# rasmusab/bayes.js

Hardware: NVIDIA H100
Metric: posterior draws/sec (chains x iters) Normal(mu,sigma) N=1024 at 1/2/4/8 H100 (higher is better)
Workload: dtype f64

## Files before the change

bayes.js_b200/csrc/amwg_jit.cuh:

```cuda
#pragma once
#include <dlfcn.h>
#include <map>
#include <mutex>
#include <sstream>

namespace jit {

struct Insn {
  int pc = 0, next = 0;
  int op = 0, a = 0;
  bool acc = false, store = false;
  int mode[4] = {AMWG_MODE_NONE, AMWG_MODE_NONE, AMWG_MODE_NONE, AMWG_MODE_NONE};
  int inl[4] = {-1, -1, -1, -1};
  int extra[3] = {0, 0, 0};
  int n_extra = 0;
  int term = -1;
  int pops = 0, pushes = 0;
};

static bool has_result(int op) {
  switch (op) {
    case AMWG_OP_ACC: case AMWG_OP_ACC_RANGE: case AMWG_OP_PLATE: case AMWG_OP_LOOP_BEGIN: case AMWG_OP_LOOP_END:
    case AMWG_OP_STORE: case AMWG_OP_END: return false;
    default: return true;
  }
}

static bool decode(const amwg_model* md, int pc, Insn& in, std::string& err) {
  const int32_t* code = md->code;
  const int n = md->n_code;
  auto need = [&](int k) { if (pc + k > n) { err = "program runs past the end of the code"; return false; } return true; };
  in = Insn();
  in.pc = pc;
  if (!need(1)) return false;
  const unsigned w = (unsigned)code[pc++];
  in.op = (int)(w & 0xff);
  in.acc = (w >> 16) & 1;
  in.store = (w & AMWG_STORE_FLAG) != 0;
  in.a = (int)(w >> 18);
  if (in.op < 0 || in.op >= AMWG_OP__COUNT) { err = "unknown opcode"; return false; }
  int used[4] = {0, 0, 0, 0};
  if (in.op == AMWG_OP_PLATE) {
    if (in.a >= md->n_plates) { err = "plate index out of range"; return false; }
    const int kind = md->plates[in.a].kind;
    if (kind == AMWG_PLATE_NORM_IID) { used[0] = used[1] = 1; }
    else if (kind == AMWG_PLATE_BERN_IID || kind == AMWG_PLATE_NORM_GROUPED) { used[0] = 1; }
  } else {
    for (int k = 0; k < 4; ++k) used[k] = ((w >> (8 + 2 * k)) & 3) != AMWG_MODE_NONE;
  }
  for (int k = 3; k >= 0; --k) {
    if (!used[k]) continue;
    const int m = (w >> (8 + 2 * k)) & 3;
    in.mode[k] = m;
    if (m == AMWG_MODE_STACK) in.pops++;
    else if (m == AMWG_MODE_NONE) { err = "plate operand without a mode"; return false; }
    else { if (!need(1)) return false; in.inl[k] = code[pc++]; }
  }
  auto take = [&](int k) { if (!need(k)) return false; for (int j = 0; j < k; ++j) in.extra[in.n_extra++] = code[pc++]; return true; };
  switch (in.op) {
    case AMWG_OP_DATA: if (!take(1)) return false; break;
    case AMWG_OP_DATA_I: if (!take(2)) return false; break;
    case AMWG_OP_COMP_I: if (!take(3)) return false; break;
    case AMWG_OP_PLATE_SS: case AMWG_OP_ACC_RANGE: case AMWG_OP_LOOP_BEGIN: if (!take(1)) return false; break;
    case AMWG_OP_LOOP_END: if (!take(1)) return false; in.pops++; break;
    case AMWG_OP_ACC: case AMWG_OP_STORE: in.pops++; break;
    default: break;
  }
  if (has_result(in.op)) {
    if (in.acc) { if (in.store) { if (!need(1)) return false; in.term = code[pc++]; } }
    else in.pushes = 1;
  } else if (in.op == AMWG_OP_PLATE && in.store) {
    if (!need(1)) return false;
    in.term = code[pc++];
  }
  in.next = pc;
  return true;
}

static bool decode_program(const amwg_model* md, int pc, std::vector<Insn>& out, int* max_depth, std::string& err) {
  out.clear();
  int depth = 0, deepest = 0;
  if (pc < 0 || pc >= md->n_code) { err = "program offset out of range"; return false; }
  for (int guard = 0; guard < md->n_code + 1; ++guard) {
    Insn in;
    if (!decode(md, pc, in, err)) return false;
    depth -= in.pops;
    if (depth < 0) { err = "operand stack underflow"; return false; }
    depth += in.pushes;
    deepest = std::max(deepest, depth);
    out.push_back(in);
    if (in.op == AMWG_OP_END) { if (max_depth) *max_depth = deepest; return true; }
    pc = in.next;
  }
  err = "program has no END";
  return false;
}

static std::string lit(double v) {
  if (v != v) return "CUDART_NAN";
  if (v == INFINITY) return "CUDART_INF";
  if (v == -INFINITY) return "(-CUDART_INF)";
  char buf[64];
  snprintf(buf, sizeof buf, "%a", v);
  std::string s(buf);
  if (v < 0 || (v == 0 && std::signbit(v))) s = "(" + s + ")";
  return s;
}
static std::string istr(long long v) { return std::to_string(v); }
static std::string bits(double v) {
  long long b;
  memcpy(&b, &v, 8);
  return std::to_string(b) + "LL";
}

struct Plan {
  int threads = 128, minblocks = 7;
  int n_res = 0;
  std::vector<int> res_col, res_off, res_bytes;
  std::vector<int> col_smem_off;
  int stream_col = -1;
  int ring_off = 0, ring_stages = 4, ring_tile = 1024;
  int ws_smem = 0, ws_off = 0;
  unsigned smem_bytes = 0;
  std::vector<int> bern_mask_off;
};

struct Source {
  bool full = false;
  std::string generated;
  std::string prelude;
  Plan plan;
};

static const int kMaxGeneratedInsns = 6000;
static const unsigned kResidentBudget = 64u * 1024u;
static const unsigned kJitWsSmemLimit = 20u * 1024u;

struct Emitter {
  std::ostringstream os;
  std::map<std::string, std::string> cse;
  std::vector<std::string> stk;
  std::vector<std::map<std::string, std::string>> scopes;
  int nv = 0;
  std::string tmp(const std::string& rhs) {
    auto it = cse.find(rhs);
    if (it != cse.end()) return it->second;
    std::string name = "v" + std::to_string(nv++);
    os << "    const double " << name << " = " << rhs << ";\n";
    cse[rhs] = name;
    return name;
  }
};

struct Inst {
  std::vector<Insn> ins;
// ... 368 lines not shown
  tables << "__device__ __forceinline__ int jp_type(int p) { return JP_TYPE[p]; }\n"
            "__device__ __forceinline__ int jp_ncomp(int p) { return JP_NCOMP[p]; }\n"
            "__device__ __forceinline__ int jp_dim0(int p) { return JP_DIM0[p]; }\n"
            "__device__ __forceinline__ int jp_off(int p) { return JP_OFF[p]; }\n"
            "__device__ __forceinline__ double jp_lower(int p) { return __longlong_as_double(JP_LOWER[p]); }\n"
            "__device__ __forceinline__ double jp_upper(int p) { return __longlong_as_double(JP_UPPER[p]); }\n";
}


static std::string build_source(const amwg_model* md, const std::vector<double>& consts, unsigned long long n_chains, int sm_count,
                                double norm_c0, Source& src) {
  if (!md->comp_prog || md->n_terms <= 0 || md->stat_prog < 0) return "the model has no pre-evaluated statistics";
  if (md->n_variant_comps > 0) return "variant programs";
  const int D = md->n_comp, P = md->n_params, NT = md->n_terms;
  if (D > 65535 || P > 255) return "too many components / parameters";
  int max_dim0 = 1;
  for (int p = 0; p < P; ++p) {
    if (md->params[p].type == AMWG_BINARY) return "binary parameter";
    if (md->params[p].n_comp > 1) max_dim0 = std::max(max_dim0, std::max(md->params[p].dim0, 2));
  }
  std::string err;

  std::vector<Insn> stat;
  if (!decode_program(md, md->stat_prog, stat, nullptr, err)) return "stat_prog: " + err;
  struct StatEntry { int q, slot, comp; size_t first, last; bool simple; };
  std::vector<StatEntry> entries;
  {
    size_t start = 0;
    for (size_t i = 0; i < stat.size(); ++i) {
      if (stat[i].op == AMWG_OP_END) break;
      if (stat[i].op != AMWG_OP_PLATE_SS) continue;
      StatEntry e{stat[i].a, stat[i].extra[0], -1, start, i, false};
      if (e.q < 0 || e.q >= md->n_plates || md->plates[e.q].kind != AMWG_PLATE_NORM_IID) return "stat_prog refers to a plate that is not NORM_IID";
      if (e.slot < 0 || e.slot >= NT) return "statistic slot out of range";
      if (i == start && stat[i].mode[0] == AMWG_MODE_COMP) { e.simple = true; e.comp = stat[i].inl[0]; if (e.comp < 0 || e.comp >= D) return "component out of range"; }
      entries.push_back(e);
      start = i + 1;
    }
  }
  if (entries.empty()) return "no plate statistics";

  Plan& pl = src.plan;
  pl = Plan();
  pl.col_smem_off.assign(md->n_columns, -1);
  std::vector<char> col_used(md->n_columns, 0);
  for (const auto& e : entries) {
    const int c = md->plates[e.q].col[0];
    if (c < 0 || c >= md->n_columns) return "plate column out of range";
    const amwg_plate& p = md->plates[e.q];
    if (p.iparam[2] < 0 || (long long)p.iparam[2] + p.n > md->columns[c].n) return "plate runs past its column";
    col_used[c] = 1;
  }
  unsigned off = 0;
  std::vector<int> big;
  for (int c = 0; c < md->n_columns; ++c) {
    if (!col_used[c]) continue;
    const unsigned bytes = pad16(std::max<size_t>(sizeof(double) * (size_t)md->columns[c].n, 16));
    if (off + bytes <= kResidentBudget) {
      pl.col_smem_off[c] = (int)off; pl.res_col.push_back(c); pl.res_off.push_back((int)off); pl.res_bytes.push_back((int)bytes);
      off += bytes;
    } else big.push_back(c);
  }
  pl.n_res = (int)pl.res_col.size();
  if (big.size() > 1) return "more than one column exceeds shared memory";
  std::vector<StatEntry> r_entries, s_entries, x_entries;
  for (const auto& e : entries) {
    const int c = md->plates[e.q].col[0];
    const bool resident = pl.col_smem_off[c] >= 0;
    if (e.simple) (resident ? r_entries : s_entries).push_back(e);
    else { if (!resident) return "a plate with an expression mean lies on a streamed column"; x_entries.push_back(e); }
  }
  int s_begin = 0, s_total = 0;
  if (!big.empty()) {
    pl.stream_col = big[0];
    if (s_entries.empty()) return "streamed column without plates";
    std::stable_sort(s_entries.begin(), s_entries.end(), [&](const StatEntry& a, const StatEntry& b) { return md->plates[a.q].iparam[2] < md->plates[b.q].iparam[2]; });
    s_begin = md->plates[s_entries[0].q].iparam[2];
    if (s_begin & 1) return "streamed plates start at an odd offset";
    int cur = s_begin;
    for (const auto& e : s_entries) {
      const amwg_plate& p = md->plates[e.q];
      if (p.iparam[2] != cur || p.n <= 0) return "streamed plates do not tile their column";
      cur += p.n;
    }
    s_total = cur - s_begin;
    pl.ring_off = (int)off;
    off += (unsigned)(pl.ring_stages * pl.ring_tile * 8);
  }
  {
    const size_t per_thread = sizeof(double) * (size_t)(2 * NT + 3 * D) + sizeof(unsigned short) * (size_t)D;
    std::string e = choose_shape(pl, off, per_thread, n_chains, sm_count);
    if (!e.empty()) return e;
  }

  std::ostringstream tables, funcs;
  int table_counter = 0;
  GenCtx gc;
  gc.md = md; gc.consts = &consts; gc.tables = &tables; gc.table_counter = &table_counter;
  std::vector<std::vector<Insn>> progs(D);
  std::map<std::string, std::vector<int>> classes_by_sig;
  std::vector<std::string> sig_order;
  int total_insns = 0;
  for (int c = 0; c < D; ++c) {
    std::vector<Insn> full;
    if (!decode_program(md, md->comp_prog[c], full, nullptr, err)) return "comp_prog: " + err;
    for (const Insn& in : full) if (in.op != AMWG_OP_ACC_RANGE) progs[c].push_back(in);
    std::string sg = signature(progs[c]);
    if (!classes_by_sig.count(sg)) sig_order.push_back(sg);
    classes_by_sig[sg].push_back(c);
  }
  std::vector<int> cls_of(D, 0), mem_of(D, 0);
  funcs << "namespace amwg {\n";
  std::ostringstream step;
  step << "__device__ __forceinline__ bool jit_step(const int c, const double prop, const double coin, double* __restrict__ wk, const unsigned long long ws,\n"
          "                                         double* __restrict__ sp, const unsigned long long ss) {\n";
  bool need_mem = false;
  struct ClassCode { std::string mem, body, stage, commit, hcommit; };
  std::vector<ClassCode> cls_code;
  bool hoist = sig_order.size() > 1;
  int n_cv = 0;
  for (size_t k = 0; k < sig_order.size(); ++k) {
    const std::vector<int>& members = classes_by_sig[sig_order[k]];
    std::vector<Inst> inst;
    for (size_t m = 0; m < members.size(); ++m) {
      Inst it; it.ins = progs[members[m]]; it.moved = members[m];
      inst.push_back(it);
      cls_of[members[m]] = (int)k; mem_of[members[m]] = (int)m;
    }
    ClassCode cc;
    std::string why;
    if (!emit_step_class(gc, inst, cc.body, cc.commit, &total_insns, why)) return "component program: " + why;
    if (total_insns > kMaxGeneratedInsns) return "the component programs are too long to specialise";
    if (cc.commit.empty()) return "a component touches no term";
    if (inst.size() > 1) { cc.mem = "    const int m = JMEM[c];\n"; need_mem = true; }
    std::istringstream lines(cc.commit);
    std::ostringstream stage, commit;
    int i = 0;
    for (std::string ln; std::getline(lines, ln);) {
      const size_t eq = ln.find(") = ");
      const std::string rhs = eq == std::string::npos ? "" : ln.substr(eq + 4);
      const bool named = rhs.size() > 2 && rhs[0] == 'v' && rhs.back() == ';' && rhs.find_first_not_of("0123456789", 1) == rhs.size() - 1;
      if (ln.compare(0, 7, "    TV(") != 0 || eq == std::string::npos) { hoist = false; break; }
      if (rhs.compare(0, 3, "TC(") == 0) { commit << ln << "\n"; continue; }
      if (!named) { hoist = false; break; }
      stage << "    cv[" << i << "] = " << rhs << "\n";
      commit << ln.substr(0, eq + 4) << "cv[" << i << "];\n";
      ++i;
    }
    n_cv = std::max(n_cv, i);
    cc.stage = stage.str();
    cc.hcommit = commit.str();
    cls_code.push_back(cc);
  }
  if (hoist) {
    step << "  double dl = 0.0;\n";
    if (n_cv > 0) step << "  double cv[" << n_cv << "];\n";
    step << "  switch (JCLS[c]) {\n";
    for (size_t k = 0; k < cls_code.size(); ++k) step << "  case " << k << ": {\n" << cls_code[k].mem << cls_code[k].body << cls_code[k].stage << "    break;\n  }\n";
    step << "  default: return false;\n  }\n";
    step << "  if (!(js_exp(dl) > coin)) return false;              // Metropolis accept (mcmc.js:527-534): strict >, NaN rejects\n";
    step << "  ST(c) = prop;\n  switch (JCLS[c]) {\n";
    for (size_t k = 0; k < cls_code.size(); ++k) step << "  case " << k << ": {\n" << cls_code[k].mem << cls_code[k].hcommit << "    break;\n  }\n";
    step << "  }\n  return true;\n}\n";
  }
  if (!hoist && sig_order.size() > 1) step << "  switch (JCLS[c]) {\n";
  for (size_t k = 0; !hoist && k < cls_code.size(); ++k) {
    if (sig_order.size() > 1) step << "  case " << k << ": {\n";
    else step << "  {\n";
    step << cls_code[k].mem << "    double dl = 0.0;\n" << cls_code[k].body;
    step << "    if (!(js_exp(dl) > coin)) return false;            // Metropolis accept (mcmc.js:527-534): strict >, NaN rejects\n";
    step << "    ST(c) = prop;\n" << cls_code[k].commit;
    step << "    return true;\n  }\n";
  }
  if (!hoist && sig_order.size() > 1) step << "  }\n  return false;\n";
  if (!hoist) step << "}\n";

  std::ostringstream extra;
  extra << "__device__ __forceinline__ void jit_stat_extra(unsigned char* smem, double* __restrict__ wk, const unsigned long long ws,\n"
           "                                               double* __restrict__ sp, const unsigned long long ss, const bool wr) {\n";
  for (const auto& e : x_entries) {
    Inst it;
    it.ins.assign(stat.begin() + e.first, stat.begin() + e.last);
    std::vector<Inst> inst{it};
    const Insn pss = stat[e.last];
    Emitter em;
    std::vector<Term> terms; std::vector<std::string> cands; std::vector<std::pair<int, std::string>> der;
    std::string why;
    if (!emit_range(gc, inst, 0, it.ins.size(), "m", CTX_STAT, em, terms, cands, der, why)) return "stat_prog: " + why;
    std::string mean;
    if (pss.mode[0] == AMWG_MODE_STACK) { if (em.stk.empty()) return "stat_prog: missing mean"; mean = em.stk.back(); }
    else if (pss.mode[0] == AMWG_MODE_CONST) { if (pss.inl[0] < 0 || pss.inl[0] >= md->n_consts) return "stat_prog: const out of range"; mean = lit(consts[pss.inl[0]]); }
    else mean = "BP(" + std::to_string(pss.inl[0]) + ")";
    total_insns += (int)it.ins.size();
    const amwg_plate& p = md->plates[e.q];
    const int so = pl.col_smem_off[p.col[0]] + 8 * p.iparam[2];
    extra << "  {\n" << em.os.str();
    extra << "    const double S = sum_sq_dev(reinterpret_cast<const double*>(smem + " << so << "), smem_u32(smem) + " << so << "u, " << p.n << ", " << mean << ");\n";
    extra << "    if (wr) TC(" << e.slot << ") = S;\n  }\n";
  }
  extra << "  (void)smem; (void)wk; (void)ws; (void)sp; (void)ss; (void)wr;\n}\n";

  std::ostringstream dfun;
  if (md->n_derived > 0) {
    Inst it;
    if (!decode_program(md, md->derived_prog, it.ins, nullptr, err)) return "derived_prog: " + err;
    std::vector<Inst> inst{it};
    Emitter em;
    std::vector<Term> terms; std::vector<std::string> cands; std::vector<std::pair<int, std::string>> der;
    std::string why;
    if (!emit_range(gc, inst, 0, it.ins.size(), "m", CTX_DERIVED, em, terms, cands, der, why)) return "derived program: " + why;
    dfun << "__device__ __forceinline__ void jit_derived(const double* __restrict__ sp, const unsigned long long ss, double* der) {\n" << em.os.str();
    for (auto& d : der) { if (d.first < 0 || d.first >= md->n_derived) return "derived index out of range"; dfun << "    der[" << d.first << "] = " << d.second << ";\n"; }
    dfun << "}\n";
  }

  auto int_table = [&](const char* qual, const char* name, const std::vector<long long>& v) {
    tables << qual << " " << name << "[" << std::max<size_t>(v.size(), 1) << "] = {";
    for (size_t i = 0; i < v.size(); ++i) tables << (i ? "," : "") << v[i];
    if (v.empty()) tables << "0";
    tables << "};\n";
  };
  {
    std::vector<long long> v;
    if (sig_order.size() > 1) { v.assign(cls_of.begin(), cls_of.end()); int_table("__device__ const unsigned char", "JCLS", v); }
    if (need_mem) { v.assign(mem_of.begin(), mem_of.end()); int_table("__device__ const unsigned short", "JMEM", v); }
    tables << "__device__ const long long KCB[" << std::max(md->n_consts, 1) << "] = {";
    for (int i = 0; i < md->n_consts; ++i) tables << (i ? "," : "") << bits(consts[i]);
    if (md->n_consts == 0) tables << "0LL";
    tables << "};\n#define KC(i) __longlong_as_double(KCB[i])\n";
    emit_param_tables(tables, md);
    std::vector<long long> a, b, c2, d;
    for (int k = 0; k < pl.n_res; ++k) { a.push_back(pl.res_off[k]); b.push_back(pl.res_col[k]); c2.push_back(pl.res_bytes[k]); }
    int_table("__constant__ unsigned", "JRES_OFF", a); int_table("__constant__ int", "JRES_COL", b); int_table("__constant__ unsigned", "JRES_BYTES", c2);
    a.clear(); b.clear(); c2.clear();
    for (const auto& e : r_entries) {
      const amwg_plate& p = md->plates[e.q];
      a.push_back(e.comp); b.push_back(pl.col_smem_off[p.col[0]] + 8 * p.iparam[2]); c2.push_back(p.n); d.push_back(e.slot);
    }
    int_table("__constant__ int", "JR_COMP", a); int_table("__constant__ unsigned", "JR_SOFF", b); int_table("__constant__ int", "JR_N", c2); int_table("__constant__ int", "JR_SLOT", d);
    a.clear(); b.clear(); d.clear();
    int cur = 0;
    for (const auto& e : s_entries) { cur += md->plates[e.q].n; a.push_back(e.comp); b.push_back(cur); d.push_back(e.slot); }
    int_table("__constant__ int", "JS_COMP", a); int_table("__constant__ int", "JS_END", b); int_table("__constant__ int", "JS_SLOT", d);
  }

  unsigned long long res_total = 0;
  for (int k = 0; k < pl.n_res; ++k) res_total += (unsigned)pl.res_bytes[k];
  int jblock = -1;
  for (int p = 0, best = 7; p < P; ++p) {
    const amwg_param& pa = md->params[p];
    if (pa.n_comp <= best) continue;
    bool indep = true;
    std::vector<int> owner((size_t)NT, -1);
    for (int c = pa.comp_offset; c < pa.comp_offset + pa.n_comp && indep; ++c)
      for (int k = md->touch_off[c]; k < md->touch_off[c + 1]; ++k) {
        int& o = owner[(size_t)md->touch_terms[k]];
        if (o >= 0 && o != c) { indep = false; break; }
        o = c;
      }
    if (indep) { jblock = p; best = pa.n_comp; }
  }
  const bool jblock_free = jblock >= 0 && md->params[jblock].lower == -INFINITY && md->params[jblock].upper == INFINITY;
  std::ostringstream pre;
  pre << "#define AMWG_PHILOX_INLINE 1\n";
  pre << "#define JBLOCK " << jblock << "\n#define JBLOCK_FREE " << (jblock_free ? 1 : 0) << "\n";
  pre << "#define JD " << D << "\n#define JP " << P << "\n#define JNT " << NT << "\n#define JNSUM " << md->n_sum_terms << "\n"
      << "#define JTHREADS " << pl.threads << "\n#define JMINB " << pl.minblocks << "\n#define JWS_SMEM " << pl.ws_smem << "\n#define JWS_OFF " << pl.ws_off << "\n"
      << "#define JN_DERIVED " << md->n_derived << "\n#define JMAX_DIM0 " << max_dim0 << "\n#define JMAXCOL " << kMaxColumns << "\n"
      << "#define JN_RES " << pl.n_res << "\n#define JRES_TOTAL_BYTES " << res_total << "u\n#define JN_RSTAT " << r_entries.size() << "\n"
      << "#define JSTREAM " << (pl.stream_col >= 0 ? 1 : 0) << "\n#define JS_COL " << std::max(pl.stream_col, 0) << "\n#define JS_BEGIN " << s_begin << "\n#define JS_TOTAL " << s_total << "\n"
      << "#define JN_SSTAT " << s_entries.size() << "\n#define JRING_OFF " << pl.ring_off << "u\n#define JRING_STAGES " << pl.ring_stages << "\n#define JRING_TILE " << pl.ring_tile << "\n"
      << "#define JNORM_C0 " << lit(norm_c0) << "\n#define AMWG_REAL 0\n#define AMWG_INT 1\n#define AMWG_BINARY 2\n";

  src.prelude = pre.str();
  funcs << tables.str() << step.str() << extra.str() << dfun.str() << "}  // namespace amwg\n";
  src.generated = funcs.str();
  return "";
}


static std::string build_source_full(const amwg_model* md, const std::vector<double>& consts, unsigned long long n_chains, int sm_count,
                                     double norm_c0, Source& src) {
  if (md->comp_prog && md->n_terms > 0) return "the model steps with a term cache";
  const int D = md->n_comp, P = md->n_params;
  if (D > 65535 || P > 255) return "too many components / parameters";
  int max_dim0 = 1;
  for (int p = 0; p < P; ++p) if (md->params[p].n_comp > 1) max_dim0 = std::max(max_dim0, std::max(md->params[p].dim0, 2));
  std::string err;
  Plan& pl = src.plan;
  pl = Plan();
  pl.col_smem_off.assign(md->n_columns, -1);
  unsigned off = 0;
  for (int c = 0; c < md->n_columns; ++c) {
    const unsigned bytes = pad16(std::max<size_t>(sizeof(double) * (size_t)md->columns[c].n, 16));
    if (off + bytes > kResidentBudget) return "the data does not fit in shared memory";
    pl.col_smem_off[c] = (int)off; pl.res_col.push_back(c); pl.res_off.push_back((int)off); pl.res_bytes.push_back((int)bytes);
    off += bytes;
  }
  pl.n_res = (int)pl.res_col.size();
  pl.bern_mask_off.assign(std::max(md->n_plates, 0), -1);
  std::vector<long long> bm_plate;
  for (int q = 0; q < md->n_plates; ++q) {
    const amwg_plate& pq = md->plates[q];
    if (pq.kind != AMWG_PLATE_BERN_IID || pq.n < 1 || pq.col[0] < 0 || pq.col[0] >= md->n_columns) continue;
    if (pq.iparam[2] < 0 || (long long)pq.iparam[2] + pq.n > md->columns[pq.col[0]].n) return "a plate runs past its column";
    off = (unsigned)pad16(off);
    pl.bern_mask_off[q] = (int)off; bm_plate.push_back(q);
    off += 4u * (unsigned)((pq.n + 31) / 32 + 1);
  }
  { std::string e = choose_shape(pl, off, sizeof(double) * (size_t)D, n_chains, sm_count); if (!e.empty()) return e; }

  std::ostringstream tables, funcs;
  int table_counter = 0, total_insns = 0;
  GenCtx gc;
  gc.md = md; gc.consts = &consts; gc.tables = &tables; gc.table_counter = &table_counter; gc.plan = &pl;
  const int n_var = md->n_variant_comps ? (1 << md->n_variant_comps) : 1;
  auto emit_program = [&](int pc, const std::string& name, bool derived) -> std::string {
    Inst it;
    if (!decode_program(md, pc, it.ins, nullptr, err)) return "program: " + err;
    total_insns += (int)it.ins.size();
    if (total_insns > kMaxGeneratedInsns) return "the programs are too long to specialise";
    std::vector<Inst> inst{it};
    Emitter em;
    std::vector<Term> terms; std::vector<std::string> cands; std::vector<std::pair<int, std::string>> der;
    std::string why;
    if (!emit_range(gc, inst, 0, it.ins.size(), "m", derived ? CTX_DERIVED : CTX_FULL, em, terms, cands, der, why)) return why;
    if (!em.scopes.empty()) return "unterminated loop";
    if (derived) {
      funcs << "__device__ __forceinline__ void " << name << "(unsigned char* smem, const double* __restrict__ sp, const unsigned long long ss, double* der) {\n" << em.os.str();
      for (auto& d : der) { if (d.first < 0 || d.first >= md->n_derived) return std::string("derived index out of range"); funcs << "    der[" << d.first << "] = " << d.second << ";\n"; }
      funcs << "  (void)smem;\n}\n";
    } else {
      funcs << "__device__ " << (it.ins.size() > 600 ? "__noinline__" : "__forceinline__") << " double " << name
            << "(unsigned char* smem, const double* __restrict__ sp, const unsigned long long ss, const int moved, const double val) {\n    double lp = 0.0;\n"
            << em.os.str() << "    (void)smem;\n    return lp;\n}\n";
    }
    return "";
  };
  for (int v = 0; v < n_var; ++v) {
    const int pc = md->n_variant_comps ? md->variant_logpost[v] : md->logpost_prog;
    std::string e = emit_program(pc, "jit_prog_" + std::to_string(v), false);
    if (!e.empty()) return "log_post: " + e;
  }
  if (md->n_derived > 0)
    for (int v = 0; v < n_var; ++v) {
      const int pc = md->n_variant_comps ? (md->variant_derived ? md->variant_derived[v] : -1) : md->derived_prog;
      if (pc < 0) return "a configuration has no derived program";
      std::string e = emit_program(pc, "jit_der_" + std::to_string(v), true);
      if (!e.empty()) return "derived: " + e;
    }
  auto variant_expr = [&](bool with_moved) {
    std::string e = "0";
    for (int k = 0; k < md->n_variant_comps; ++k) {
      const std::string c = std::to_string(md->variant_comps[k]);
      e += " | ((" + (with_moved ? "CM(" + c + ")" : "ST(" + c + ")") + " != 0.0) ? " + std::to_string(1 << k) + " : 0)";
    }
    return e;
  };
  funcs << "__device__ __forceinline__ double jit_logpost(unsigned char* smem, const double* __restrict__ sp, const unsigned long long ss, const int moved, const double val) {\n";
  if (n_var == 1) funcs << "  return jit_prog_0(smem, sp, ss, moved, val);\n";
  else {
    funcs << "  switch (" << variant_expr(true) << ") {\n";
    for (int v = 0; v < n_var; ++v) funcs << "    case " << v << ": return jit_prog_" << v << "(smem, sp, ss, moved, val);\n";
    funcs << "  }\n  return CUDART_NAN;\n";
  }
  funcs << "}\n";
  if (md->n_derived > 0) {
    funcs << "__device__ __forceinline__ void jit_derived(unsigned char* smem, const double* __restrict__ sp, const unsigned long long ss, double* der) {\n";
    if (n_var == 1) funcs << "  jit_der_0(smem, sp, ss, der);\n";
    else {
      funcs << "  switch (" << variant_expr(false) << ") {\n";
      for (int v = 0; v < n_var; ++v) funcs << "    case " << v << ": jit_der_" << v << "(smem, sp, ss, der); break;\n";
      funcs << "  }\n";
    }
    funcs << "}\n";
  }
  std::ostringstream t2;
  emit_param_tables(t2, md);
  auto int_table = [&](const char* qual, const char* name, const std::vector<long long>& v) {
    t2 << qual << " " << name << "[" << std::max<size_t>(v.size(), 1) << "] = {";
    for (size_t i = 0; i < v.size(); ++i) t2 << (i ? "," : "") << v[i];
    if (v.empty()) t2 << "0";
    t2 << "};\n";
  };
  std::vector<long long> a1, b1, c1;
  for (int k = 0; k < pl.n_res; ++k) { a1.push_back(pl.res_off[k]); b1.push_back(pl.res_col[k]); c1.push_back(pl.res_bytes[k]); }
  int_table("__constant__ unsigned", "JRES_OFF", a1); int_table("__constant__ int", "JRES_COL", b1); int_table("__constant__ unsigned", "JRES_BYTES", c1);
  {
    std::vector<long long> bd, bn, bo;
    for (long long q : bm_plate) {
      const amwg_plate& pq = md->plates[q];
      bd.push_back(pl.col_smem_off[pq.col[0]] + 8 * pq.iparam[2]); bn.push_back(pq.n); bo.push_back(pl.bern_mask_off[q]);
    }
    int_table("__constant__ unsigned", "JBERN_DATA", bd); int_table("__constant__ int", "JBERN_N", bn); int_table("__constant__ unsigned", "JBERN_MASK", bo);
  }
  t2 << "__device__ const long long KCB[" << std::max(md->n_consts, 1) << "] = {";
  for (int i = 0; i < md->n_consts; ++i) t2 << (i ? "," : "") << bits(consts[i]);
  if (md->n_consts == 0) t2 << "0LL";
  t2 << "};\n#define KC(i) __longlong_as_double(KCB[i])\n";
  unsigned long long res_total = 0;
  for (int k = 0; k < pl.n_res; ++k) res_total += (unsigned)pl.res_bytes[k];
  std::ostringstream pre;
  pre << "#define JFULL 1\n#define JD " << D << "\n#define JP " << P << "\n#define JTHREADS " << pl.threads << "\n#define JMINB " << pl.minblocks
      << "\n#define JWS_SMEM " << pl.ws_smem << "\n#define JWS_OFF " << pl.ws_off << "\n#define JN_DERIVED " << md->n_derived << "\n#define JMAX_DIM0 " << max_dim0
      << "\n#define JMAXCOL " << kMaxColumns << "\n#define JN_BERN " << bm_plate.size() << "\n#define JN_RES " << pl.n_res << "\n#define JRES_TOTAL_BYTES " << res_total << "u\n#define JNORM_C0 " << lit(norm_c0)
      << "\n#define AMWG_REAL 0\n#define AMWG_INT 1\n#define AMWG_BINARY 2\n";
  src.prelude = pre.str();
  src.generated = "namespace amwg {\n#define LD(o) lds_f64_sa(smem_u32(smem) + (o))\n" + t2.str() + tables.str() + funcs.str() + "}  // namespace amwg\n";
  src.full = true;
  return "";
}

typedef int nvrtcResult_t;
typedef struct _nvrtcProgram* nvrtcProgram_t;
struct Nvrtc {
  void* h = nullptr;
  nvrtcResult_t (*CreateProgram)(nvrtcProgram_t*, const char*, const char*, int, const char* const*, const char* const*) = nullptr;
  nvrtcResult_t (*DestroyProgram)(nvrtcProgram_t*) = nullptr;
  nvrtcResult_t (*CompileProgram)(nvrtcProgram_t, int, const char* const*) = nullptr;
  nvrtcResult_t (*GetCUBINSize)(nvrtcProgram_t, size_t*) = nullptr;
  nvrtcResult_t (*GetCUBIN)(nvrtcProgram_t, char*) = nullptr;
  nvrtcResult_t (*GetProgramLogSize)(nvrtcProgram_t, size_t*) = nullptr;
  nvrtcResult_t (*GetProgramLog)(nvrtcProgram_t, char*) = nullptr;
  const char* (*GetErrorString)(nvrtcResult_t) = nullptr;
  std::string error;
};

static Nvrtc* nvrtc() {
// ... 113 lines not shown
```

bayes.js_b200/csrc/amwg_jit_kernel.cuh:

```cuda
#pragma once

namespace amwg {

struct JitArgs {
  ChainArrays a;
  SweepArgs sa;
  const double* col[JMAXCOL];
  const unsigned char* adapting;
};

#define TV(t) wk[(unsigned long long)(t) * ws]
#define TC(t) wk[(unsigned long long)(JNT + (t)) * ws]
#define BP(c) wk[(unsigned long long)(2 * JNT + (c)) * ws]
#define BC(c) wk[(unsigned long long)(2 * JNT + JD + (c)) * ws]
#define ST(c) sp[(unsigned long long)(c) * ss]

}

#include "amwg_jit_generated.inc"

namespace amwg {

extern "C" __global__ void __launch_bounds__(JTHREADS, JMINB) amwg_jit_sweep(const __grid_constant__ JitArgs A) {
  extern __shared__ __align__(16) unsigned char smem[];
  __shared__ __align__(8) unsigned long long bar_res;
#if JSTREAM
  __shared__ __align__(8) unsigned long long ring_full[JRING_STAGES];
#endif
  const ChainArrays& a = A.a;
  const SweepArgs& sa = A.sa;
  const unsigned long long C = a.C;
  const unsigned long long tid = (unsigned long long)blockIdx.x * blockDim.x + threadIdx.x;
  const bool valid = tid < C;
  const unsigned long long chain = valid ? tid : C - 1;
  const unsigned long long gchain = a.first_chain + chain;

  if (threadIdx.x == 0) {
    mbar_init(&bar_res, 1);
#if JSTREAM
    for (int k = 0; k < JRING_STAGES; ++k) mbar_init(&ring_full[k], 1);
#endif
    asm volatile("fence.mbarrier_init.release.cluster;" ::: "memory");
  }
  __syncthreads();
#if JN_RES > 0
  if (threadIdx.x == 0) {
    mbar_expect_tx(&bar_res, JRES_TOTAL_BYTES);
#pragma unroll
    for (int k = 0; k < JN_RES; ++k) tma_bulk_g2s(smem + JRES_OFF[k], A.col[JRES_COL[k]], JRES_BYTES[k], &bar_res);
  }
  mbar_wait(&bar_res, 0);
#endif

#if JWS_SMEM
  double* wk = reinterpret_cast<double*>(smem + JWS_OFF) + threadIdx.x;
  const unsigned long long ws = JTHREADS, ss = JTHREADS;
  double* sp = wk + (unsigned long long)(2 * JNT + 2 * JD) * ws;
  unsigned short* vq = reinterpret_cast<unsigned short*>(smem + JWS_OFF + (size_t)(2 * JNT + 3 * JD) * JTHREADS * sizeof(double)) + threadIdx.x;
  for (int t = 0; t < JNT; ++t) TV(t) = a.tval[(unsigned long long)t * C + chain];
  for (int c = 0; c < JD; ++c) ST(c) = a.state[(unsigned long long)c * C + chain];
  const bool wr = true;
#else
  double* wk = a.tval + chain;
  const unsigned long long ws = C, ss = C;
  double* sp = a.state + chain;
  unsigned short* vq = a.vseq + chain;
  const bool wr = valid;
#endif

  RandomStream g;
  g.init(a.rng_n[chain]);
  unsigned long long perm = a.perm[chain];
#if JMAX_DIM0 > 1
  unsigned char order[JMAX_DIM0 < kLocalOrder ? JMAX_DIM0 : kLocalOrder];
#endif
#if JSTREAM
  unsigned ring_fills = 0;
#endif

  long long rec_phase = sa.record ? sa.sample_i0 % sa.thin : 0;
  long long row = sa.record ? (sa.sample_i0 + sa.thin - 1) / sa.thin : 0;
  for (long long s = 0; s < sa.n_sweeps; ++s) {
    if (sa.record) {
      const bool rec_now = rec_phase == 0;
      if (++rec_phase == sa.thin) rec_phase = 0;
      if (rec_now && valid) {
#if JN_DERIVED > 0
        double der[JN_DERIVED];
        bool have_der = false;
#endif
        for (int j = 0; j < sa.n_monitor; ++j) {
          const int e = sa.monitor[j];
          double v;
          if (e < JD) {
            v = ST(e);
          } else {
#if JN_DERIVED > 0
            if (!have_der) { jit_derived(sp, ss, der); have_der = true; }
            v = der[e - JD];
#else
            v = CUDART_NAN;
#endif
          }
          sa.out[((unsigned long long)row * sa.n_monitor + j) * C + chain] = v;
        }
      }
      if (rec_now) ++row;
    }
#if JP > 1
    for (int i = JP - 1; i > 0; --i) {
      const int j = (int)floor(g.next(a.seed, gchain) * (i + 1));
      perm_swap(a, perm, chain, i, j, valid);
    }
#endif
    int pos = 0;
#pragma unroll 1
    for (int slot = 0; slot < JP; ++slot) {
      const int p = (JP > 1) ? perm_get(a, perm, chain, slot) : 0;
      const int n_comp = jp_ncomp(p), off = jp_off(p), ptype = jp_type(p);
      const double lower = jp_lower(p), upper = jp_upper(p);
#if JMAX_DIM0 > 1
      const int dim0 = jp_dim0(p);
      const int inner = n_comp / dim0;
      if (n_comp > 1) {
        for (int i = 0; i < dim0; ++i) ord_set(a, order, chain, dim0, i, i, valid);
        for (int i = dim0 - 1; i > 0; --i) {
          const int j = (int)floor(g.next(a.seed, gchain) * (i + 1));
          const int t = ord_get(a, order, chain, dim0, i);
          ord_set(a, order, chain, dim0, i, ord_get(a, order, chain, dim0, j), valid);
          ord_set(a, order, chain, dim0, j, t, valid);
        }
      }
#endif
#pragma unroll 1
      for (int r = 0; r < n_comp; ++r, ++pos) {
        int c = off;
#if JMAX_DIM0 > 1
        if (n_comp > 1) c += ord_get(a, order, chain, dim0, r / inner) * inner + (r % inner);
#endif
#if JBLOCK >= 0 && JBLOCK_FREE
        if (p == JBLOCK) {
          const double z = js_rnorm_ratio(g, a.seed, gchain);
          const double coin = g.next(a.seed, gchain);
          if (wr) { BP(c) = z; BC(c) = coin; }
          continue;
        }
#endif
        const double cur = ST(c);
        double prop = js_rnorm(g, a.seed, gchain, cur, a.psd[(unsigned long long)c * C + chain]);
        if (ptype == AMWG_INT) prop = js_round(prop);
        const bool inb = !(prop < lower || prop > upper);
        const double coin = inb ? g.next(a.seed, gchain) : -1.0;
        if (wr) {
          BP(c) = inb ? prop : cur;
          BC(c) = coin;
          vq[(unsigned long long)pos * ws] = (unsigned short)c;
        }
      }
    }
#if JBLOCK >= 0 && JBLOCK_FREE
    {
      const int n_b = jp_ncomp(JBLOCK), off_b = jp_off(JBLOCK);
      const bool is_int = jp_type(JBLOCK) == AMWG_INT;
#pragma unroll 4
      for (int r = 0; r < n_b; ++r) {
        const int c = off_b + r;
        double prop = BP(c) * a.psd[(unsigned long long)c * C + chain] + ST(c);
        if (is_int) prop = js_round(prop);
        if (wr) BP(c) = prop;
      }
    }
#endif
#if JN_RSTAT > 0
#pragma unroll 1
    for (int k = 0; k < JN_RSTAT; ++k) {
      const double mean = BP(JR_COMP[k]);
      const unsigned sa0 = smem_u32(smem) + JR_SOFF[k];
      const double S = sum_sq_dev(reinterpret_cast<const double*>(smem + JR_SOFF[k]), sa0, JR_N[k], mean);
      if (wr) TC(JR_SLOT[k]) = S;
    }
#endif
    jit_stat_extra(smem, wk, ws, sp, ss, wr);
#if JSTREAM
    {
      const int nt = (JS_TOTAL + JRING_TILE - 1) / JRING_TILE;
      const double* gx = A.col[JS_COL] + JS_BEGIN;
      __syncthreads();
      if (threadIdx.x == 0)
        for (int t = 0; t < JRING_STAGES - 1 && t < nt; ++t) {
          const unsigned st = (ring_fills + (unsigned)t) % JRING_STAGES;
          const int cnt = min(JRING_TILE, JS_TOTAL - t * JRING_TILE);
          const unsigned bytes = (unsigned)((cnt * 8 + 15) & ~15);
          mbar_expect_tx(&ring_full[st], bytes);
          tma_bulk_g2s(smem + JRING_OFF + st * (JRING_TILE * 8), gx + (size_t)t * JRING_TILE, bytes, &ring_full[st]);
        }
      int pk = 0;
      double S = 0.0;
      double mean = BP(JS_COMP[0]);
      int pend = JS_END[0];
#pragma unroll 1
      for (int t = 0; t < nt; ++t) {
        __syncthreads();
        if (threadIdx.x == 0 && t + JRING_STAGES - 1 < nt) {
          const int t2 = t + JRING_STAGES - 1;
          const unsigned st = (ring_fills + (unsigned)t2) % JRING_STAGES;
          const int cnt = min(JRING_TILE, JS_TOTAL - t2 * JRING_TILE);
          const unsigned bytes = (unsigned)((cnt * 8 + 15) & ~15);
          mbar_expect_tx(&ring_full[st], bytes);
          tma_bulk_g2s(smem + JRING_OFF + st * (JRING_TILE * 8), gx + (size_t)t2 * JRING_TILE, bytes, &ring_full[st]);
        }
        const unsigned f = ring_fills + (unsigned)t;
        const unsigned st = f % JRING_STAGES;
        mbar_wait(&ring_full[st], (f / JRING_STAGES) & 1u);
        const int lo = t * JRING_TILE, hi = min(lo + JRING_TILE, JS_TOTAL);
        int p0 = lo;
        while (p0 < hi) {
          const int e = min(pend, hi);
          const unsigned boff = JRING_OFF + st * (JRING_TILE * 8) + 8u * (unsigned)(p0 - lo);
          S = S + sum_sq_dev(reinterpret_cast<const double*>(smem + boff), smem_u32(smem) + boff, e - p0, mean);
          p0 = e;
          if (p0 == pend) {
            if (wr) TC(JS_SLOT[pk]) = S;
            ++pk;
            S = 0.0;
            if (pk < JN_SSTAT) { mean = BP(JS_COMP[pk]); pend = JS_END[pk]; }
          }
        }
      }
      ring_fills += (unsigned)nt;
    }
#endif
#if JBLOCK < 0
    {
      int c_next = (int)vq[0];
      double coin_next = BC(c_next), prop_next = BP(c_next);
#pragma unroll 1
      for (int i = 0; i < JD; ++i) {
        const int c = c_next;
        const double coin = coin_next, prop = prop_next;
        if (i + 1 < JD) {
          c_next = (int)vq[(unsigned long long)(i + 1) * ws];
          coin_next = BC(c_next); prop_next = BP(c_next);
        }
        if (!wr || coin < 0.0) continue;
        if (jit_step(c, prop, coin, wk, ws, sp, ss) && valid && A.adapting[c])
          atomicAdd(&a.acc[(unsigned long long)c * C + chain], 1);
      }
    }
#else
    {
      int pos_b = 0;
      for (int slot = 0; slot < JP; ++slot) if (((JP > 1) ? perm_get(a, perm, chain, slot) : 0) == JBLOCK) pos_b = slot;
#pragma unroll 1
      for (int part = 0; part < 3; ++part) {
        if (part == 1) {
          const int n_b = jp_ncomp(JBLOCK), off_b = jp_off(JBLOCK);
          double coin_next = BC(off_b), prop_next = BP(off_b);
#pragma unroll 1
          for (int r = 0; r < n_b; ++r) {
            const int c = off_b + r;
            const double coin = coin_next, prop = prop_next;
            if (r + 1 < n_b) { coin_next = BC(c + 1); prop_next = BP(c + 1); }
            if (!wr || coin < 0.0) continue;
            if (jit_step(c, prop, coin, wk, ws, sp, ss) && valid && A.adapting[c]) atomicAdd(&a.acc[(unsigned long long)c * C + chain], 1);
          }
          continue;
        }
        const int lo = part == 0 ? 0 : pos_b + 1, hi = part == 0 ? pos_b : JP;
        int pos0 = 0;
#pragma unroll 1
        for (int slot = 0; slot < JP; ++slot) {
          const int p = (JP > 1) ? perm_get(a, perm, chain, slot) : 0;
          const int n_comp = jp_ncomp(p);
          if (slot >= lo && slot < hi) {
            int c_next = (int)vq[(unsigned long long)pos0 * ws];
            double coin_next = BC(c_next), prop_next = BP(c_next);
#pragma unroll 1
            for (int r = 0; r < n_comp; ++r) {
              const int c = c_next;
              const double coin = coin_next, prop = prop_next;
              if (r + 1 < n_comp) {
                c_next = (int)vq[(unsigned long long)(pos0 + r + 1) * ws];
                coin_next = BC(c_next); prop_next = BP(c_next);
              }
              if (!wr || coin < 0.0) continue;
              if (jit_step(c, prop, coin, wk, ws, sp, ss) && valid && A.adapting[c])
                atomicAdd(&a.acc[(unsigned long long)c * C + chain], 1);
            }
          }
          pos0 += n_comp;
        }
      }
    }
#endif
  }
  if (valid) {
    a.rng_n[chain] = g.n;
    a.perm[chain] = perm;
#if JWS_SMEM
    for (int t = 0; t < JNT; ++t) a.tval[(unsigned long long)t * C + chain] = TV(t);
    for (int c = 0; c < JD; ++c) a.state[(unsigned long long)c * C + chain] = ST(c);
#endif
  }
}

}
```

Before: 4.651 billion.

## Hoist proposal-only expensive subexpressions out of the step and cache current-state twins

The JIT code generator scans each singleton class's step body for expressions that depend only on the proposal (divisions, js_/ld_ calls). It emits a jit_hoist_props pass that evaluates them once per sweep into free term-cache rows before the statistic/streaming phase, and rewrites the step body to read those rows. Matching expressions evaluated at the current state are cached too: they are initialised at kernel start and updated on accept by copying the proposal row. This takes divisions and transcendentals off the serial per-component Metropolis path, at the cost of extra shared-memory traffic, more generated-code complexity, and fragile text-based expression parsing.

```diff
diff --git a/bayes.js_b200/csrc/amwg_jit.cuh b/bayes.js_b200/csrc/amwg_jit.cuh
--- a/bayes.js_b200/csrc/amwg_jit.cuh
+++ b/bayes.js_b200/csrc/amwg_jit.cuh
@@ -1,6 +1,7 @@
 #pragma once
 #include <dlfcn.h>
 #include <map>
+#include <set>
 #include <mutex>
 #include <sstream>
 
@@ -675,6 +676,119 @@
     cc.hcommit = commit.str();
     cls_code.push_back(cc);
   }
+  std::string hoist_src;
+  if (hoist && pl.ws_smem) {
+    struct Line { std::string name, expr; };
+    auto parse = [](const std::string& body) {
+      std::vector<Line> out;
+      std::istringstream in(body);
+      for (std::string ln; std::getline(in, ln);) {
+        const std::string head = "    const double ";
+        const size_t eq = ln.find(" = ");
+        if (ln.compare(0, head.size(), head) != 0 || eq == std::string::npos || ln.back() != ';') { out.push_back({"", ln}); continue; }
+        out.push_back({ln.substr(head.size(), eq - head.size()), ln.substr(eq + 3, ln.size() - eq - 4)});
+      }
+      return out;
+    };
+    auto prop_only = [](const std::string& e, const std::set<std::string>& ok, bool& refs_named) {
+      refs_named = false;
+      for (size_t i = 0; i < e.size();) {
+        const char ch = e[i];
+        if (isdigit((unsigned char)ch) || (ch == '.' && i + 1 < e.size() && isdigit((unsigned char)e[i + 1]))) {
+          while (i < e.size() && (isalnum((unsigned char)e[i]) || e[i] == '.' ||
+                                  ((e[i] == '+' || e[i] == '-') && (e[i - 1] == 'p' || e[i - 1] == 'P' || e[i - 1] == 'e' || e[i - 1] == 'E')))) ++i;
+          continue;
+        }
+        if (isalpha((unsigned char)ch) || ch == '_') {
+          size_t j = i;
+          while (j < e.size() && (isalnum((unsigned char)e[j]) || e[j] == '_')) ++j;
+          const std::string id = e.substr(i, j - i);
+          const bool call = j < e.size() && e[j] == '(';
+          if (ok.count(id)) refs_named = true;
+          else if (!(id == "prop" || id == "CUDART_NAN" || id == "CUDART_INF" || id == "JNORM_C0" || (call && (id == "KC" || id.compare(0, 3, "js_") == 0 || id.compare(0, 3, "ld_") == 0)))) return false;
+          i = j;
+          continue;
+        }
+        ++i;
+      }
+      return true;
+    };
+    auto subst_prop = [](const std::string& e, const std::string& by) {
+      std::string out;
+      for (size_t i = 0; i < e.size();) {
+        if ((isalpha((unsigned char)e[i]) || e[i] == '_') && (i == 0 || !(isalnum((unsigned char)e[i - 1]) || e[i - 1] == '_'))) {
+          size_t j = i;
+          while (j < e.size() && (isalnum((unsigned char)e[j]) || e[j] == '_')) ++j;
+          const std::string id = e.substr(i, j - i);
+          out += id == "prop" ? by : id;
+          i = j;
+          continue;
+        }
+        out += e[i++];
+      }
+      return out;
+    };
+    std::set<int> used;
+    bool ok = true;
+    for (const auto& e : entries) used.insert(e.slot);
+    for (const auto& cc : cls_code)
+      for (const std::string* t : {&cc.body, &cc.commit})
+        for (size_t q = t->find("TC("); q != std::string::npos; q = t->find("TC(", q + 3)) {
+          const size_t r = t->find(')', q);
+          const std::string ix = t->substr(q + 3, r - q - 3);
+          if (ix.empty() || ix.find_first_not_of("0123456789") != std::string::npos) ok = false;
+          else used.insert(std::stoi(ix));
+        }
+    std::vector<int> free_rows;
+    for (int t = NT - 1; ok && t >= 0; --t) if (!used.count(t)) free_rows.push_back(t);
+    std::vector<std::vector<Line>> lines(cls_code.size());
+    for (size_t k = 0; k < cls_code.size(); ++k) lines[k] = parse(cls_code[k].body);
+    std::ostringstream props, init;
+    for (int c = 0; c < D && !free_rows.empty(); ++c) {
+      const int k = cls_of[c];
+      if (classes_by_sig[sig_order[k]].size() != 1) continue;
+      std::set<std::string> named;
+      std::ostringstream eval, store;
+      for (Line& l : lines[k]) {
+        if (l.name.empty()) continue;
+        bool refs = false;
+        if (!prop_only(l.expr, named, refs)) continue;
+        named.insert(l.name);
+        eval << "    const double " << l.name << " = " << l.expr << ";\n";
+        if (free_rows.empty() || (l.expr.find('/') == std::string::npos && l.expr.find("js_") == std::string::npos && l.expr.find("ld_") == std::string::npos)) continue;
+        std::vector<Line*> twins;
+        if (!refs) {
+          const std::string at = subst_prop(l.expr, "ST(" + std::to_string(c) + ")");
+          for (auto& ls : lines) for (Line& o : ls) if (!o.name.empty() && o.expr == at) twins.push_back(&o);
+        }
+        if (!twins.empty() && free_rows.size() < 2) twins.clear();
+        const int rp = free_rows.back();
+        free_rows.pop_back();
+        store << "    TC(" << rp << ") = " << l.name << ";\n";
+        if (!twins.empty()) {
+          const int rc = free_rows.back();
+          free_rows.pop_back();
+          init << "  TC(" << rc << ") = " << twins[0]->expr << ";\n";
+          for (Line* o : twins) o->expr = "TC(" + std::to_string(rc) + ")";
+          cls_code[k].hcommit += "    TC(" + std::to_string(rc) + ") = TC(" + std::to_string(rp) + ");\n";
+        }
+        l.expr = "TC(" + std::to_string(rp) + ")";
+      }
+      if (!store.str().empty())
+        props << "  if (BC(" << c << ") >= 0.0) {                 // in bounds: the step will be evaluated\n    const double prop = BP(" << c
+              << ");\n" << eval.str() << store.str() << "  }\n";
+    }
+    if (!props.str().empty()) {
+      for (size_t k = 0; k < cls_code.size(); ++k) {
+        std::string b;
+        for (const Line& l : lines[k]) b += l.name.empty() ? l.expr + "\n" : "    const double " + l.name + " = " + l.expr + ";\n";
+        cls_code[k].body = b;
+      }
+      hoist_src = "__device__ __forceinline__ void jit_hoist_props(double* __restrict__ wk, const unsigned long long ws) {\n" + props.str() +
+                  "}\n__device__ __forceinline__ void jit_hoist_init(double* __restrict__ wk, const unsigned long long ws, const double* __restrict__ sp,\n"
+                  "                                               const unsigned long long ss) {\n" + init.str() + "}\n";
+    }
+  }
   if (hoist) {
     step << "  double dl = 0.0;\n";
     if (n_cv > 0) step << "  double cv[" << n_cv << "];\n";
@@ -795,8 +909,9 @@
       << "#define JN_SSTAT " << s_entries.size() << "\n#define JRING_OFF " << pl.ring_off << "u\n#define JRING_STAGES " << pl.ring_stages << "\n#define JRING_TILE " << pl.ring_tile << "\n"
       << "#define JNORM_C0 " << lit(norm_c0) << "\n#define AMWG_REAL 0\n#define AMWG_INT 1\n#define AMWG_BINARY 2\n";
 
+  if (!hoist_src.empty()) pre << "#define JHOIST 1\n";
   src.prelude = pre.str();
-  funcs << tables.str() << step.str() << extra.str() << dfun.str() << "}  // namespace amwg\n";
+  funcs << tables.str() << step.str() << extra.str() << dfun.str() << hoist_src << "}  // namespace amwg\n";
   src.generated = funcs.str();
   return "";
 }
diff --git a/bayes.js_b200/csrc/amwg_jit_kernel.cuh b/bayes.js_b200/csrc/amwg_jit_kernel.cuh
--- a/bayes.js_b200/csrc/amwg_jit_kernel.cuh
+++ b/bayes.js_b200/csrc/amwg_jit_kernel.cuh
@@ -60,6 +60,9 @@
   for (int t = 0; t < JNT; ++t) TV(t) = a.tval[(unsigned long long)t * C + chain];
   for (int c = 0; c < JD; ++c) ST(c) = a.state[(unsigned long long)c * C + chain];
   const bool wr = true;
+#ifdef JHOIST
+  jit_hoist_init(wk, ws, sp, ss);
+#endif
 #else
   double* wk = a.tval + chain;
   const unsigned long long ws = C, ss = C;
@@ -170,6 +173,9 @@
         if (wr) BP(c) = prop;
       }
     }
+#endif
+#ifdef JHOIST
+    jit_hoist_props(wk, ws);
 #endif
 #if JN_RSTAT > 0
 #pragma unroll 1
```

Measured after the change: 4.733 billion (median of 6 runs). 1.02x the previous value.
